# egbariajad/GNN-Accelerated-LAP-Warm-Start-Pipeline

Measured on AMD Instinct MI355X. Metric: LAP instances/sec (whole node), n=2048 warm-start pipeline, higher is better.
Workload: dtype f64

## Files before the change

gnn-accelerated-lap-warm-start-pipeline_amd/csrc/device_utils.hpp:

```cpp
#pragma once

#include <hip/hip_runtime.h>
#include <stdint.h>

namespace lapwarm {

constexpr int kWave = 64;
constexpr int kMaxWaves = 16;
constexpr double kLarge = 1000000.0;

constexpr int kFlagHasViolation = 1;
constexpr int kFlagInfeasible = 2;
constexpr int kFlagProjected = 4;

__device__ __forceinline__ void pin(double &x) { asm volatile("" : "+v"(x)); }

__device__ __forceinline__ int lo32(double x) { return (int)(__double_as_longlong(x) & 0xffffffffLL); }
__device__ __forceinline__ int hi32(double x) { return (int)(__double_as_longlong(x) >> 32); }
__device__ __forceinline__ double mk_f64(int lo, int hi)
{
    return __longlong_as_double(((long long)hi << 32) | (unsigned int)lo);
}

__device__ __forceinline__ int uni(int x) { return __builtin_amdgcn_readfirstlane(x); }
// ... 47 lines not shown
__device__ __forceinline__ double readlane_f64(double x, int l)
{
    const long long b = __double_as_longlong(x);
    const int lo = __builtin_amdgcn_readlane((int)(b & 0xffffffffLL), l);
    const int hi = __builtin_amdgcn_readlane((int)(b >> 32), l);
    return __longlong_as_double(((long long)hi << 32) | (unsigned int)lo);
}
__device__ __forceinline__ double readlane(double x, int l) { return readlane_f64(x, l); }

struct Top2 {
    double a1;
    int i1;
    double a2;
    int i2;
};

__device__ __forceinline__ Top2 top2_empty()
{
    Top2 t;
    t.a1 = pos_inf();
    t.i1 = 0x7fffffff;
    t.a2 = pos_inf();
    t.i2 = 0x7fffffff;
    return t;
}

__device__ __forceinline__ void top2_push(Top2 &t, double a, int i)
{
    const bool first = pair_less(a, i, t.a1, t.i1);
    const bool second = pair_less(a, i, t.a2, t.i2);
    const double n2a = first ? t.a1 : (second ? a : t.a2);
    const int n2i = first ? t.i1 : (second ? i : t.i2);
    t.a1 = first ? a : t.a1;
    t.i1 = first ? i : t.i1;
    t.a2 = n2a;
    t.i2 = n2i;
}

__device__ __forceinline__ Top2 top2_merge(Top2 p, Top2 q)
{
    const bool qf = pair_less(q.a1, q.i1, p.a1, p.i1);
    const double fa = qf ? q.a1 : p.a1;
    const int fi = qf ? q.i1 : p.i1;
    const double la = qf ? p.a1 : q.a1;
    const int li = qf ? p.i1 : q.i1;
    const double sa = qf ? q.a2 : p.a2;
    const int si = qf ? q.i2 : p.i2;
    const bool ls = pair_less(la, li, sa, si);
    Top2 r;
    r.a1 = fa;
    r.i1 = fi;
    r.a2 = ls ? la : sa;
    r.i2 = ls ? li : si;
    return r;
}


template <class Op>
__device__ __forceinline__ typename Op::T wave_reduce(typename Op::T v)
{
    v = Op::combine(dpp_move<kDppRowShr1, 0xf>(Op::identity(), v), v);
    v = Op::combine(dpp_move<kDppRowShr2, 0xf>(Op::identity(), v), v);
    v = Op::combine(dpp_move<kDppRowShr4, 0xf>(Op::identity(), v), v);
    v = Op::combine(dpp_move<kDppRowShr8, 0xf>(Op::identity(), v), v);
    v = Op::combine(dpp_move<kDppRowBcast15, 0xa>(Op::identity(), v), v);
    v = Op::combine(dpp_move<kDppRowBcast31, 0xc>(Op::identity(), v), v);
    return readlane(v, kWave - 1);
}

template <class Op>
__device__ __forceinline__ typename Op::T row_reduce(typename Op::T v)
{
    v = Op::combine(dpp_move<kDppRowShr1, 0xf>(Op::identity(), v), v);
    v = Op::combine(dpp_move<kDppRowShr2, 0xf>(Op::identity(), v), v);
    v = Op::combine(dpp_move<kDppRowShr4, 0xf>(Op::identity(), v), v);
    v = Op::combine(dpp_move<kDppRowShr8, 0xf>(Op::identity(), v), v);
    return readlane(v, 15);
}

struct MinF64 {
    using T = double;
    static __device__ __forceinline__ T identity() { return pos_inf(); }
    static __device__ __forceinline__ T combine(T o, T v) { return dmin(v, o); }
};
struct NanMinF64 : MinF64 {
    static __device__ __forceinline__ T combine(T o, T v) { return nmin(v, o); }
};
struct FminF64 : MinF64 {
    static __device__ __forceinline__ T combine(T o, T v) { return __builtin_fmin(v, o); }
};
struct MaxF64 {
    using T = double;
    static __device__ __forceinline__ T identity() { return -pos_inf(); }
    static __device__ __forceinline__ T combine(T o, T v) { return (o > v) ? o : v; }
};
struct MinI32 {
    using T = int;
    static __device__ __forceinline__ T identity() { return 0x7fffffff; }
    static __device__ __forceinline__ T combine(T o, T v) { return (o < v) ? o : v; }
};
struct SumI32 {
    using T = int;
    static __device__ __forceinline__ T identity() { return 0; }
    static __device__ __forceinline__ T combine(T o, T v) { return v + o; }
};
struct MinU64 {
    using T = unsigned long long;
    static __device__ __forceinline__ T identity() { return ~0ull; }
    static __device__ __forceinline__ T combine(T o, T v) { return (o < v) ? o : v; }
};
__device__ __forceinline__ unsigned f32_key(float x)
{
    if (x != x) return 0xffffffffu;
    unsigned b = __float_as_uint(x);
    if (b == 0x80000000u) b = 0u;
    return (b & 0x80000000u) ? ~b : (b | 0x80000000u);
}

__device__ __forceinline__ double wave_min(double v) { return wave_reduce<MinF64>(v); }
__device__ __forceinline__ double wave_max(double v) { return wave_reduce<MaxF64>(v); }
__device__ __forceinline__ int wave_min_i32(int v) { return wave_reduce<MinI32>(v); }
__device__ __forceinline__ int wave_sum_i32(int v) { return wave_reduce<SumI32>(v); }

template <int CTRL, int ROW_MASK>
__device__ __forceinline__ Top2 top2_step(Top2 t)
{
    Top2 o;
    o.a1 = dpp_move<CTRL, ROW_MASK>(pos_inf(), t.a1);
    o.i1 = dpp_move<CTRL, ROW_MASK>(0x7fffffff, t.i1);
    o.a2 = dpp_move<CTRL, ROW_MASK>(pos_inf(), t.a2);
    o.i2 = dpp_move<CTRL, ROW_MASK>(0x7fffffff, t.i2);
    return top2_merge(t, o);
}
__device__ __forceinline__ Top2 wave_top2(Top2 t)
{
    t = top2_step<kDppRowShr1, 0xf>(t);
    t = top2_step<kDppRowShr2, 0xf>(t);
    t = top2_step<kDppRowShr4, 0xf>(t);
    t = top2_step<kDppRowShr8, 0xf>(t);
    t = top2_step<kDppRowBcast15, 0xa>(t);
    t = top2_step<kDppRowBcast31, 0xc>(t);
    Top2 r;
    r.a1 = readlane_f64(t.a1, kWave - 1);
    r.i1 = __builtin_amdgcn_readlane(t.i1, kWave - 1);
    r.a2 = readlane_f64(t.a2, kWave - 1);
    r.i2 = __builtin_amdgcn_readlane(t.i2, kWave - 1);
    return r;
}

__device__ __forceinline__ double wave_sum_f64(double v)
{
#pragma unroll
    for (int m = 32; m >= 1; m >>= 1) v += __shfl_xor(v, m, kWave);
    return v;
}

template <int CTRL, int ROW_MASK>
__device__ __forceinline__ void scan_step_min_pair(double &v, int &i)
{
    const double ov = dpp_move<CTRL, ROW_MASK>(pos_inf(), v);
    const int oi = dpp_move<CTRL, ROW_MASK>(0x7fffffff, i);
    if (pair_less(ov, oi, v, i)) {
        v = ov;
        i = oi;
    }
}

__device__ __forceinline__ void wave_excl_prefix_min_pair(double &v, int &idx, int lane, double *tv, int *ti)
{
    double iv = v;
    int ii = idx;
    scan_step_min_pair<kDppRowShr1, 0xf>(iv, ii);
    scan_step_min_pair<kDppRowShr2, 0xf>(iv, ii);
    scan_step_min_pair<kDppRowShr4, 0xf>(iv, ii);
    scan_step_min_pair<kDppRowShr8, 0xf>(iv, ii);
    scan_step_min_pair<kDppRowBcast15, 0xa>(iv, ii);
    scan_step_min_pair<kDppRowBcast31, 0xc>(iv, ii);
    {
        const long long b = __double_as_longlong(iv);
        const int lo = __builtin_amdgcn_readlane((int)(b & 0xffffffffLL), kWave - 1);
        const int hi = __builtin_amdgcn_readlane((int)(b >> 32), kWave - 1);
        *tv = __longlong_as_double(((long long)hi << 32) | (unsigned int)lo);
        *ti = __builtin_amdgcn_readlane(ii, kWave - 1);
    }
    const double pv = __shfl_up(iv, 1, kWave);
    const int pi = __shfl_up(ii, 1, kWave);
    v = (lane == 0) ? pos_inf() : pv;
    idx = (lane == 0) ? 0x7fffffff : pi;
}

struct BlockExchange {
    double d[2][kMaxWaves * 4];
    double bcast[2];
    int i[2][kMaxWaves * 4];
};

struct Arr2 {
    double a1, vj1, a2;
    int i1, y1, i2, y2;
};

__device__ __forceinline__ Arr2 arr2_empty()
{
    Arr2 t;
    t.a1 = t.a2 = pos_inf();
    t.vj1 = 0.0;
    t.i1 = t.i2 = 0x7fffffff;
    t.y1 = t.y2 = -1;
    return t;
}

__device__ __forceinline__ void arr2_push(Arr2 &t, double a, int i, double vj, int yj)
{
    const bool first = pair_less(a, i, t.a1, t.i1);
    const bool second = pair_less(a, i, t.a2, t.i2);
    t.a2 = first ? t.a1 : (second ? a : t.a2);
    t.i2 = first ? t.i1 : (second ? i : t.i2);
    t.y2 = first ? t.y1 : (second ? yj : t.y2);
    t.a1 = first ? a : t.a1;
    t.i1 = first ? i : t.i1;
    t.vj1 = first ? vj : t.vj1;
    t.y1 = first ? yj : t.y1;
}

template <int WIDTH>
__device__ __forceinline__ double lanes_min(double v)
{
    static_assert(WIDTH == 64 || WIDTH == 16, "a whole wave or one row");
    if constexpr (WIDTH == 64)
        return wave_reduce<MinF64>(v);
    else
        return row_reduce<MinF64>(v);
}

template <int WIDTH>
__device__ __forceinline__ Arr2 arr2_reduce_lanes(const Arr2 &t)
{
    constexpr int last = WIDTH - 1;
    const unsigned long long lanes = (WIDTH == 64) ? ~0ull : 0xffffull;
    const double m1 = lanes_min<WIDTH>(t.a1);
    const unsigned long long k1 = __ballot(t.a1 == m1) & lanes;
    const int l1 = k1 ? __builtin_ctzll(k1) : 0;
    Arr2 r;
    r.a1 = readlane_f64(t.a1, l1);
    r.vj1 = readlane_f64(t.vj1, l1);
    r.i1 = __builtin_amdgcn_readlane(t.i1, l1);
    r.y1 = __builtin_amdgcn_readlane(t.y1, l1);
    const int lane = threadIdx.x & (kWave - 1);
    const double c2 = ((lane & last) == l1) ? t.a2 : t.a1;
    const int c2i = ((lane & last) == l1) ? t.i2 : t.i1;
    const int c2y = ((lane & last) == l1) ? t.y2 : t.y1;
    const double m2 = lanes_min<WIDTH>(c2);
    const unsigned long long k2 = __ballot(c2 == m2) & lanes;
    const int l2 = k2 ? __builtin_ctzll(k2) : 0;
    r.a2 = readlane_f64(c2, l2);
    r.i2 = __builtin_amdgcn_readlane(c2i, l2);
    r.y2 = __builtin_amdgcn_readlane(c2y, l2);
    return r;
}

struct BlockCtx {
    int tid, lane, wave, nwaves;
    int parity;
    BlockExchange *ex;

    __device__ __forceinline__ void init(BlockExchange *e)
    {
        tid = threadIdx.x;
        lane = tid & (kWave - 1);
        wave = tid >> 6;
        nwaves = (blockDim.x + kWave - 1) >> 6;
        parity = 0;
        ex = e;
    }

    __device__ __forceinline__ double &slot(int p, int w, double) { return ex->d[p][w]; }
    __device__ __forceinline__ int &slot(int p, int w, int) { return ex->i[p][w]; }
    __device__ __forceinline__ unsigned long long &slot(int p, int w, unsigned long long)
    {
        return reinterpret_cast<unsigned long long &>(ex->d[p][w]);
    }

    template <class Op>
    __device__ __forceinline__ typename Op::T reduce(typename Op::T v)
    {
        v = wave_reduce<Op>(v);
        const int p = parity;
        parity ^= 1;
        if (lane == 0) slot(p, wave, v) = v;
        __syncthreads();
        const int w = lane & (kMaxWaves - 1);
        return row_reduce<Op>((w < nwaves) ? slot(p, w, v) : Op::identity());
    }

    template <class Op = MinF64>
    __device__ __forceinline__ double min_f64(double v) { return reduce<Op>(v); }
    __device__ __forceinline__ int min_i32(int v) { return reduce<MinI32>(v); }
    __device__ __forceinline__ int sum_i32(int v) { return reduce<SumI32>(v); }

    __device__ __forceinline__ double max_f64(double v)
    {
        v = wave_max(v);
        const int p = parity;
        parity ^= 1;
        if (lane == 0) ex->d[p][wave] = v;
        __syncthreads();
// ... 136 lines not shown
```

gnn-accelerated-lap-warm-start-pipeline_amd/csrc/jv_solver.hip:

```cpp
#include <string.h>

#include "device_utils.hpp"
#include "jv_solver.hpp"
#include "solve_plan.hpp"

namespace lapwarm {

namespace {

struct EventSlot {
    int j, p, i, a;
};

constexpr int kRecEvents = 4;

struct alignas(16) Ctrl {
    double level;
    int hi;
    int target;
    alignas(16) EventSlot rec[2][kRecEvents];
    alignas(16) int a_pub[2][kRecEvents];
    int tie_find;
    int ev_total[2];
    int first_fire;
    int nfree;
    int err;
    int head_j, head_i;
    int free_pos[2];
};
struct ArrState {
    unsigned arr_current, arr_rr;
    int arr_new_free, arr_fwd, arr_iters, arr_fast, arr_err;
};
static_assert(sizeof(ArrState) <= sizeof(EventSlot) * 2 * kRecEvents, "ArrState is overlaid on Ctrl::rec");

constexpr int kSentinelIdx = 0x7ffffffe;
constexpr int kEmptyIdx = 0x7fffffff;

#ifdef LAPWARM_STAMPS
__device__ __forceinline__ unsigned long long stamp_now()
{
    unsigned long long t;
    asm volatile("s_memtime %0\n\ts_waitcnt lgkmcnt(0)" : "=s"(t)::"memory");
    return t;
}
#ifndef LAPWARM_STAMP_GROUPS
#define LAPWARM_STAMP_GROUPS 7
#endif
#define STAMP_G(g, var) const unsigned long long var = ((LAPWARM_STAMP_GROUPS) & (g)) ? stamp_now() : 0ull
#ifndef LAPWARM_FIND_MASK
#define LAPWARM_FIND_MASK 0x1ff
#endif
#define STAMP_FI(bit, var) const unsigned long long var = (((LAPWARM_STAMP_GROUPS) & 1) && ((LAPWARM_FIND_MASK) >> (bit) & 1)) ? stamp_now() : 0ull
#define STAMP(var) STAMP_G(1, var)
#define STAMPR(var) STAMP_G(2, var)
#define STAMPP(var) STAMP_G(4, var)
#define STAMP_ADD(slot, t1, t0) stamps[slot] += (long long)((t1) - (t0))
#define STAMP_INC(slot) stamps[slot] += 1
#else
#define STAMP(var)
#define STAMPR(var)
#define STAMPP(var)
#define STAMP_FI(bit, var)
#define STAMP_ADD(slot, t1, t0)
#define STAMP_INC(slot)
#endif

template <int CH, int LDSL, int TB, bool RAGGED = false>
struct Solver {
    static constexpr bool LDS_STATE = LDSL > 0 && LDSL != 8;
    static constexpr bool ROWLDS = LDSL == 8;
    static constexpr bool PF = ROWLDS;
    static constexpr int kCacheLimit = (TB <= 256) ? 16 : ((TB <= 512) ? 32 : 4);
    static constexpr int kCacheLimitY = (TB <= 256) ? 16 : 2;
    const double *C;
    int n, W;
    int ldc;
    double *dist, *v;
    int *order, *pred, *y, *x, *fr;
    int *ring;
    int ring_count;
    unsigned char *slots;
    int slot_bytes;
    int nslots;
    uint32_t *evt, *sbits, *used;
    uint32_t *evb;
    int Wpad;
    int *evl;
    int *tmpcol;
    Ctrl *ctrl;
    BlockCtx bc;
    long long scan_elems, init_elems, colred_elems;
    int paths, finds, scan_steps, arr_iters, transfer_rows, arr_fired;
    int step_id;
    int ctrl_seen0, ctrl_seen1, ctrl_find_seq;
    int err;
#ifdef LAPWARM_STAMPS
    long long stamps[kStampSlots];
#endif

    __device__ __forceinline__ int base() const { return bc.tid * CH; }

    __device__ __forceinline__ void ring_push(int row)
    {
        if (ring && (unsigned)row < (unsigned)n) {
            if (bc.tid == 0) {
                const int gen = (ring_count >> 6) + 1;
                __hip_atomic_store(&ring[2 + (ring_count & (kRingSlots - 1))], (gen << 16) | row, __ATOMIC_RELAXED,
                                   __HIP_MEMORY_SCOPE_AGENT);
            }
            ++ring_count;
        }
    }
    __device__ __forceinline__ void ring_push_scan(int lo, int hi)
    {
        if (!ring) return;
        int cnt = hi - lo - 1;
        if (cnt <= 0) return;
        cnt = (cnt < kRingSlots - 2) ? cnt : kRingSlots - 2;
        if (bc.wave == 0 && bc.lane < cnt) {
            const int j = order[lo + 1 + bc.lane];
            const int i = ((unsigned)j < (unsigned)n) ? y[j] : -1;
            const int c = ring_count + bc.lane;
            const int gen = (c >> 6) + 1;
            const int word = (gen << 16) | (((unsigned)i < (unsigned)n) ? i : 0xffff);
            __hip_atomic_store(&ring[2 + (c & (kRingSlots - 1))], word, __ATOMIC_RELAXED, __HIP_MEMORY_SCOPE_AGENT);
        }
        ring_count += cnt;
    }

    __device__ __forceinline__ void fence_if_global()
    {
        if constexpr (!LDS_STATE) __threadfence_block();
    }

    __device__ __forceinline__ void replay_find(int lo)
    {
        const int lane = bc.lane;
        const int wpl = (W + kWave - 1) / kWave;
        int mine = 0;
        for (int q = 0; q < wpl; ++q) {
            const int idx = lane * wpl + q;
            if (idx < W) mine += __popc(evt[idx]);
        }
        int incl = mine;
#pragma unroll
        for (int off = 1; off < kWave; off <<= 1) {
            const int o = __shfl_up(incl, off, kWave);
            if (lane >= off) incl += o;
        }
        const int E = __shfl(incl, kWave - 1, kWave);
        int slot = incl - mine;
        int last_strict_local = -1;
        for (int q = 0; q < wpl; ++q) {
            const int idx = lane * wpl + q;
            if (idx < W) {
                uint32_t ew = evt[idx];
                const uint32_t sw = sbits[idx];
                if (ew) {
                    evt[idx] = 0;
                    sbits[idx] = 0;
                }
                while (ew) {
                    const int bit = __builtin_ctz(ew);
                    ew &= ew - 1;
                    const int st = (sw >> bit) & 1u;
                    if (st) last_strict_local = slot;
                    evl[slot++] = ((idx << 5) + bit) | (st << 31);
                }
            }
        }
        int L = last_strict_local;
#pragma unroll
        for (int m = 32; m >= 1; m >>= 1) {
            const int o = __shfl_xor(L, m, kWave);
            L = (o > L) ? o : L;
        }
        bool early_tie = false;
        for (int i = lane; i < L; i += kWave) early_tie |= (evl[i] >= 0);
        int hi;
        if (__ballot(early_tie) != 0ull || L + 1 > kWave) {
            hi = lo + 1;
            for (int i = 0; i < E; ++i) {
                const int ev = evl[i];
                const int k = ev & 0x7fffffff;
                const int j = order[k];
                if (ev < 0) hi = lo;
                const int a = order[hi];
                if (lane == 0) {
                    order[k] = a;
                    order[hi] = j;
                }
                fence_if_global();
                ++hi;
            }
        } else {
            const int T = E - (L + 1);
            for (int base_i = 0; base_i <= L; base_i += kWave) {
                const int i = base_i + lane;
                int newcol = 0, e = 0;
                if (i <= L) {
                    e = evl[i] & 0x7fffffff;
                    newcol = order[(i == 0) ? lo : (evl[i - 1] & 0x7fffffff)];
                }
                const int lastcol = (L >= 0) ? order[evl[L] & 0x7fffffff] : 0;
                if (i <= L) order[e] = newcol;
                if (base_i == 0 && L >= 0 && lane == 0) order[lo] = lastcol;
            }
            fence_if_global();
            const int tb = L + 1;
            for (int s0 = 1; s0 <= T; s0 += kWave) {
                const int sidx = s0 + lane;
                if (sidx <= T) tmpcol[sidx] = order[evl[tb + sidx - 1] & 0x7fffffff];
            }
            fence_if_global();
            for (int s0 = 1; s0 <= T; s0 += kWave) {
                const int sidx = s0 + lane;
                if (sidx <= T) {
                    const int p0 = lo + sidx;
                    int tpos = evl[tb + sidx - 1] & 0x7fffffff;
                    bool is_tie;
                    {
                        int lo_i = 1, hi_i = sidx;
                        while (lo_i < hi_i) {
                            const int mid = (lo_i + hi_i) >> 1;
                            if ((evl[tb + mid - 1] & 0x7fffffff) < p0)
                                lo_i = mid + 1;
                            else
                                hi_i = mid;
                        }
                        is_tie = ((evl[tb + lo_i - 1] & 0x7fffffff) == p0);
                    }
                    if (!is_tie) {
                        const int col = order[p0];
                        int p = tpos;
                        int guard = 0;
                        while (p <= lo + T && guard++ < n) p = evl[tb + (p - lo) - 1] & 0x7fffffff;
                        order[p] = col;
                    }
                }
            }
            fence_if_global();
            for (int s0 = 1; s0 <= T; s0 += kWave) {
                const int sidx = s0 + lane;
                if (sidx <= T) order[lo + sidx] = tmpcol[sidx];
            }
            fence_if_global();
            hi = lo + 1 + T;
        }
        int best = -1;
        for (int kk = lo + lane; kk < hi; kk += kWave) {
            if (y[order[kk]] < 0) best = kk;
        }
#pragma unroll
        for (int m = 32; m >= 1; m >>= 1) {
            const int o = __shfl_xor(best, m, kWave);
            best = (o > best) ? o : best;
        }
        const int target = (best >= 0) ? order[best] : -1;
        const int head_j = order[lo];
        const double level = dist[head_j];
        const int head_i = y[head_j];
        if (lane == 0) {
            ctrl->hi = hi;
            ctrl->target = target;
            ctrl->level = level;
            ctrl->head_j = head_j;
            ctrl->head_i = head_i;
        }
    }

    __device__ __forceinline__ void replay_scan(int hi, int par)
    {
        const int lane = bc.lane;
        uint32_t *evb = this->evb + (size_t)par * Wpad;
        int target = -1;
        const int fp = uni(ctrl->free_pos[par]);
        if (fp != 0x7fffffff && lane == 0) ctrl->free_pos[par] = 0x7fffffff;
        for (int wbase = 0; wbase < W; wbase += kWave) {
            const int idx = wbase + lane;
            uint32_t ew = 0;
            if (idx < W) {
                ew = evb[idx];
                if (ew) evb[idx] = 0;
            }
            unsigned long long mask = __ballot(ew != 0);
            while (mask && target < 0) {
                const int l = __builtin_ctzll(mask);
                mask &= mask - 1;
                uint32_t e = __shfl(ew, l, kWave);
                while (e && target < 0) {
                    const int bit = __builtin_ctz(e);
                    e &= e - 1;
                    const int k = ((wbase + l) << 5) + bit;
                    const int j = order[k];
                    if (k == fp) {
                        target = j;
                    } else {
                        const int a = order[hi];
                        if (lane == 0) {
                            order[k] = a;
                            order[hi] = j;
                        }
                        fence_if_global();
                        ++hi;
                    }
                }
            }
        }
        if (lane == 0) {
            ctrl->hi = hi;
            ctrl->target = target;
        }
    }

    __device__ __forceinline__ int find_path(int start)
    {
        const int b0 = base();
        const int wordi = b0 >> 5, shift = b0 & 31;
        STAMPP(tpath);
        constexpr bool CACHE_V = CH <= kCacheLimit;
        double dk[CH], vr[CACHE_V ? CH : 1];
        constexpr bool CACHE_Y = CH <= kCacheLimitY;
        int jr[CH], yr[CACHE_Y ? CH : 1];
        {
            const double *row = C + (size_t)start * (RAGGED ? ldc : n);
            double c0[CH];
#pragma unroll
            for (int r = 0; r < CH; ++r) {
                const int k = b0 + r;
                jr[r] = (k < n) ? k : n - 1;
                c0[r] = row[jr[r]];
            }
#pragma unroll
            for (int r = 0; r < CH; ++r) pin(c0[r]);
#pragma unroll
            for (int r = 0; r < CH; ++r) {
                const int k = b0 + r;
                const double vk = v[jr[r]];
                if constexpr (CACHE_V) {
                    vr[r] = vk;
                    if constexpr (CACHE_Y) yr[r] = y[jr[r]];
                }
                const double val = c0[r] - vk;
                dk[r] = (k < n) ? val : pos_inf();
                if (k < n) {
                    order[k] = k;
                    pred[k] = start;
                    dist[k] = val;
                }
            }
        }
        paths++;
        init_elems += n;
        int lo = 0, hi = 0, ready = 0, target = -1;
        int head_j = 0, head_i = 0;
        STAMPP(tp0);
        STAMP_ADD(8, tp0, tpath);
        int seen0 = ctrl_seen0, seen1 = ctrl_seen1;
        int find_seq = ctrl_find_seq;
        int app_pos = -1, app_j = 0, app_i = 0, app_j1 = 0, app_i1 = 0;
        bool app_two = false;
        constexpr bool kFastMulti = CH <= 4;
        bool pf_have = false;
        int pf_slot = 0;
        double level = 0.0;
        int guard = 0;
        while (target < 0) {
            if (lo == hi) {
                STAMP_FI(0, tf0);
                ready = lo;
                ++find_seq;
                double tv = pos_inf();
                int tp = 0x7fffffff;
#pragma unroll
                for (int r = 0; r < CH; ++r) {
                    const int k = b0 + r;
                    if (k >= lo && k < n && (k == lo || dk[r] < tv)) {
                        tv = dk[r];
                        tp = k;
                    }
                }
                double runv = tv, wtv;
                int runp = tp, wtp;
                wave_excl_prefix_min_pair(runv, runp, bc.lane, &wtv, &wtp);
                const int xp = bc.parity;
                bc.parity ^= 1;
                if (bc.lane == 0) {
                    bc.ex->d[xp][bc.wave] = wtv;
                    bc.ex->i[xp][bc.wave] = wtp;
                }
                STAMP_FI(1, tfa);
                STAMP_ADD(9, tfa, tf0);
                __syncthreads();
                STAMP_FI(2, tfb);
                STAMP_ADD(10, tfb, tfa);
                double totv;
                int totp;
                {
                    const int w = bc.lane & (kMaxWaves - 1);
                    double av = (w < bc.nwaves) ? bc.ex->d[xp][w] : pos_inf();
                    int ap = (w < bc.nwaves) ? bc.ex->i[xp][w] : 0x7fffffff;
                    scan_step_min_pair<kDppRowShr1, 0xf>(av, ap);
                    scan_step_min_pair<kDppRowShr2, 0xf>(av, ap);
                    scan_step_min_pair<kDppRowShr4, 0xf>(av, ap);
                    scan_step_min_pair<kDppRowShr8, 0xf>(av, ap);
                    totv = readlane_f64(av, kMaxWaves - 1);
                    totp = __builtin_amdgcn_readlane(ap, kMaxWaves - 1);
                    if (bc.wave > 0) {
                        const int wl = uni(bc.wave) - 1;
                        const double pv = readlane_f64(av, wl);
                        const int pp = __builtin_amdgcn_readlane(ap, wl);
                        if (pair_less(pv, pp, runv, runp)) {
                            runv = pv;
                            runp = pp;
                        }
                    }
                }
                STAMP_FI(3, tfc);
                uint32_t eb = 0, sb = 0;
                bool tie = false;
                int prevpos[CH];
                double prevval[CH];
#pragma unroll
                for (int r = 0; r < CH; ++r) {
                    const int k = b0 + r;
                    prevpos[r] = -1;
                    prevval[r] = 0.0;
                    if (k >= lo && k < n) {
                        if (k > lo && dk[r] <= runv) {
                            eb |= 1u << r;
                            if (dk[r] < runv) {
                                sb |= 1u << r;
                                prevpos[r] = runp;
                                prevval[r] = runv;
                            } else {
                                tie = true;
                            }
                        }
                        if (k == lo || dk[r] < runv) {
                            runv = dk[r];
                            runp = k;
                        }
                    }
                }
                int prevcol[CH];
#pragma unroll
                for (int r = 0; r < CH; ++r) prevcol[r] = (prevpos[r] >= 0) ? order[prevpos[r]] : 0;
                const int min_col = uni(order[totp]);
                if (tie) ctrl->tie_find = find_seq;
                const int min_row_raw = y[min_col];
                ring_push(uni(min_row_raw));
                STAMP_FI(4, tfd);
                STAMP_ADD(11, tfd, tfc);
                __syncthreads();
                STAMP_FI(5, tfe);
                STAMP_ADD(12, tfe, tfd);
                finds++;
                if (uni(ctrl->tie_find) != find_seq) {
                    hi = lo + 1;
                    level = totv;
                    head_j = min_col;
                    head_i = uni(min_row_raw);
                    target = (head_i < 0) ? head_j : -1;
                    if (target >= 0) break;
#pragma unroll
                    for (int r = 0; r < CH; ++r) {
                        if (sb & (1u << r)) {
                            const int k = b0 + r;
                            order[k] = prevcol[r];
                            jr[r] = prevcol[r];
                            dk[r] = prevval[r];
                            if constexpr (CACHE_V) {
                                vr[r] = v[prevcol[r]];
                                if constexpr (CACHE_Y) yr[r] = y[prevcol[r]];
                            }
                        }
                    }
                    if (totp != lo && lo >= b0 && lo < b0 + CH) order[lo] = min_col;
                    STAMP_FI(6, tff);
                    STAMP_ADD(13, tff, tfe);
                } else {
                    if (eb) {
                        atomicOr(&evt[wordi], eb << shift);
                        if (sb) atomicOr(&sbits[wordi], sb << shift);
                    }
                    __syncthreads();
                    if (bc.wave == 0) replay_find(lo);
                    __syncthreads();
                    hi = uni(ctrl->hi);
                    target = uni(ctrl->target);
                    level = uni(ctrl->level);
                    head_j = uni(ctrl->head_j);
                    head_i = uni(ctrl->head_i);
                    STAMP_FI(7, tfg);
                    STAMP_ADD(14, tfg, tfe);
                    STAMP_INC(15);
                    if (target >= 0) break;
                    ring_push_scan(lo, hi);
#pragma unroll
                    for (int r = 0; r < CH; ++r) {
                        const int k = b0 + r;
                        if (k >= hi && k < n) {
                            const int j = order[k];
                            if (j != jr[r]) {
                                jr[r] = j;
                                if constexpr (CACHE_V) {
                                    vr[r] = v[j];
                                    if constexpr (CACHE_Y) yr[r] = y[j];
                                }
                                dk[r] = dist[j];
                            }
                        }
                    }
                }
                STAMP_FI(8, tf1);
                STAMP_ADD(0, tf1, tf0);
            }
            STAMPR(tr0);
            if ((unsigned)head_i >= (unsigned)n || (unsigned)head_j >= (unsigned)n) {
                err = 6;
                break;
            }
            const double *row = C + (size_t)head_i * (RAGGED ? ldc : n);
            double c[CH];
            double c_head;
            bool from_slot = false;
            if constexpr (PF) from_slot = pf_have;
            if constexpr (ROWLDS) {
                if (!from_slot) {
                    pf_slot = 0;
                    const unsigned sbase = lds_address(slots) + (unsigned)bc.wave * 1024u;
                    const int nt = (int)blockDim.x;
#pragma unroll
                    for (int q = 0; q < CH / 2; ++q) {
                        int col = q * 2 * nt + 2 * bc.tid;
                        col = (col < n - 2) ? col : n - 2;
                        dma_request16(row + col, sbase + (unsigned)q * (unsigned)nt * 16u);
                    }
                    drain();
                    __syncthreads();
                    from_slot = true;
                }
            }
            const double *srow = reinterpret_cast<const double *>(slots + (size_t)pf_slot * slot_bytes);
            if constexpr (ROWLDS) {
                c_head = srow[head_j];
            } else if (from_slot) {
#pragma unroll
                for (int r = 0; r < CH; ++r) {
                    const unsigned jc = umin_u32((unsigned)jr[r], (unsigned)(n - 1));
                    c[r] = srow[jc];
                }
                c_head = srow[head_j];
            } else {
#pragma unroll
                for (int r = 0; r < CH; ++r) {
                    const unsigned jc = umin_u32((unsigned)jr[r], (unsigned)(n - 1));
                    c[r] = row[jc];
                }
                c_head = row[head_j];
            }
            const int par = step_id & 1;
            step_id++;
            scan_steps++;
            scan_elems += (long long)(n - hi);
            if (++guard > 2 * n + 4) {
                err = 1;
                break;
            }
            const bool queued = (lo + 1 < hi);
            int nq_j = 0, nq_i = 0;
            const int fwd_pos = app_pos;
            const bool fwd_two = app_two;
            app_pos = -1;
            app_two = false;
            if (queued) {
                if (fwd_two && lo == fwd_pos) {
                    nq_j = app_j1;
                    nq_i = app_i1;
                } else if (lo + 1 == fwd_pos) {
                    nq_j = app_j;
                    nq_i = app_i;
                } else {
                    nq_j = order[lo + 1];
                    nq_i = y[nq_j];
                }
            }

            bool pf_issued = false;
            int pf_next_slot = 0;
            if constexpr (PF) {
                const int ri = uni(nq_i);
                if (queued && (unsigned)ri < (unsigned)n && nslots > 1) {
                    pf_next_slot = from_slot ? (pf_slot ^ 1) : 0;
                    const double *nrow = C + (size_t)ri * (RAGGED ? ldc : n);
                    const unsigned sbase = lds_address(slots) + (unsigned)pf_next_slot * (unsigned)slot_bytes +
                                           (unsigned)bc.wave * 1024u;
                    const int nt = (int)blockDim.x;
#pragma unroll
                    for (int q = 0; q < CH / 2; ++q) {
                        int col = q * 2 * nt + 2 * bc.tid;
                        col = (col < n - 2) ? col : n - 2;
                        dma_request16(nrow + col, sbase + (unsigned)q * (unsigned)nt * 16u);
                    }
                    pf_issued = true;
                }
            }
            if constexpr (kFastMulti) {
                if (b0 <= hi + kRecEvents - 1 && b0 + CH - 1 >= hi) {
#pragma unroll
                    for (int r = 0; r < CH; ++r) {
                        const unsigned w = (unsigned)(b0 + r - hi);
                        if (w < (unsigned)kRecEvents && b0 + r < n) ctrl->a_pub[par][w] = jr[r];
                    }
                }
            } else {
                if (hi >= b0 && hi < b0 + CH && hi < n) {
#pragma unroll
                    for (int r = 0; r < CH; ++r)
                        if (b0 + r == hi) ctrl->a_pub[par][0] = jr[r];
                }
            }
            const double v_head = v[head_j];
            if constexpr (!ROWLDS) {
#pragma unroll
                for (int r = 0; r < CH; ++r) pin(c[r]);
            }
            pin(c_head);
            STAMPR(tr1);
            STAMP_ADD(1, tr1, tr0);
            const double h = (c_head - v_head) - level;
            int my_events = 0, ev_r = -1;
            unsigned imp_bits = 0, ev_mask = 0;
#pragma unroll
            for (int r = 0; r < CH; ++r) {
                const int k = b0 + r;
                const bool act = (k >= hi) & (k < n);
                double vj;
                if constexpr (CACHE_V)
                    vj = vr[r];
                else
                    vj = v[jr[r]];
                double cr;
                if constexpr (ROWLDS)
                    cr = srow[umin_u32((unsigned)jr[r], (unsigned)(n - 1))];
                else
                    cr = c[r];
                const double cand = (cr - vj) - h;
                const bool imp = act & (cand < dk[r]);
                const bool ev = imp & (cand == level);
                dk[r] = imp ? cand : (act ? dk[r] : pos_inf());
                imp_bits |= imp ? (1u << r) : 0u;
                ev_mask |= ev ? (1u << r) : 0u;
            }
            if (imp_bits) {
#pragma unroll
                for (int r = 0; r < CH; ++r) {
                    if ((imp_bits >> r) & 1u) {
                        dist[jr[r]] = dk[r];
                        pred[jr[r]] = head_i;
                    }
                }
                if (ev_mask) {
#pragma unroll
                    for (int r = CH - 1; r >= 0; --r) {
                        if ((ev_mask >> r) & 1u) {
                            ev_r = r;
                            ++my_events;
                            const int k = b0 + r;
                            atomicOr(&evb[par * Wpad + (k >> 5)], 1u << (k & 31));
                            int yj;
                            if constexpr (CACHE_Y)
                                yj = yr[r];
                            else
                                yj = y[jr[r]];
                            if (yj < 0) atomicMin(&ctrl->free_pos[par], k);
                        }
                    }
                }
            }
            const int seen = par ? seen1 : seen0;
            if (my_events && !kFastMulti) {
                atomicAdd(&ctrl->ev_total[par], my_events);
                EventSlot sl;
                sl.j = 0;
                sl.i = 0;
#pragma unroll
                for (int r = 0; r < CH; ++r) {
                    if (r == ev_r) {
                        sl.j = jr[r];
                        if constexpr (CACHE_Y)
                            sl.i = yr[r];
                        else
                            sl.i = y[jr[r]];
                    }
                }
                sl.p = b0 + ev_r;
                sl.a = 0;
                ctrl->rec[par][0] = sl;
            }
            if (my_events && kFastMulti) {
                int slot_idx = atomicAdd(&ctrl->ev_total[par], my_events) - seen;
#pragma unroll
                for (int r = 0; r < CH; ++r) {
                    if ((ev_mask >> r) & 1u) {
                        if (slot_idx < kRecEvents) {
                            EventSlot sl;
                            sl.j = jr[r];
                            if constexpr (CACHE_Y)
                                sl.i = yr[r];
                            else
                                sl.i = y[jr[r]];
                            sl.p = b0 + r;
                            sl.a = 0;
                            ctrl->rec[par][slot_idx] = sl;
                        }
                        ++slot_idx;
                    }
                }
            }
            STAMPR(tr2);
            STAMP_ADD(2, tr2, tr1);
            if constexpr (PF) {
                if (pf_issued) drain();
                pf_have = pf_issued;
                pf_slot = pf_next_slot;
            }
            __syncthreads();
            STAMPR(tr3);
            STAMP_ADD(3, tr3, tr2);
            const int tot_raw = ctrl->ev_total[par];
            EventSlot sl = ctrl->rec[par][0];
            const int a_raw = ctrl->a_pub[par][0];
            const int tot = uni(tot_raw);
            const int cnt = tot - seen;
            if (par)
                seen1 = tot;
            else
                seen0 = tot;
            if (cnt == 0) {
                STAMP_INC(5);
                ++lo;
                if (queued) {
                    head_j = uni(nq_j);
                    head_i = uni(nq_i);
                }
            } else if (cnt == 1) {
                STAMP_INC(6);
                sl.j = uni(sl.j);
                sl.p = uni(sl.p);
                sl.i = uni(sl.i);
                sl.a = uni(a_raw);
                if ((unsigned)sl.j >= (unsigned)n || (unsigned)sl.a >= (unsigned)n || (unsigned)sl.p >= (unsigned)n ||
                    sl.i >= n) {
                    err = 8;
                    break;
                }
                if (sl.p >= b0 && sl.p < b0 + CH) {
                    evb[par * Wpad + (sl.p >> 5)] = 0;
                    if (sl.i >= 0) {
                        const double va = v[sl.a], da = dist[sl.a];
                        const int ya = y[sl.a];
#pragma unroll
                        for (int r = 0; r < CH; ++r) {
                            if (b0 + r == sl.p) {
                                jr[r] = sl.a;
                                if constexpr (CACHE_V) {
                                    vr[r] = va;
                                    if constexpr (CACHE_Y) yr[r] = ya;
                                }
                                dk[r] = da;
                            }
                        }
                        order[sl.p] = sl.a;
                        order[hi] = sl.j;
                    }
                }
                if (sl.i < 0) {
                    if (bc.tid == 0) ctrl->free_pos[par] = 0x7fffffff;
                    target = sl.j;
                    break;
                }
                app_pos = hi;
                app_j = sl.j;
                app_i = sl.i;
                ring_push(sl.i);
                ++hi;
                ++lo;
                if (queued) {
                    head_j = uni(nq_j);
                    head_i = uni(nq_i);
                } else {
                    head_j = sl.j;
                    head_i = sl.i;
                }
            } else {
                STAMP_INC(7);
                bool resolved = false;
                if (kFastMulti && cnt <= kRecEvents) {
                    const EventSlot e1 = ctrl->rec[par][1];
                    const EventSlot e2 = ctrl->rec[par][2];
                    const EventSlot e3 = ctrl->rec[par][3];
                    const int4 aw = *reinterpret_cast<const int4 *>(ctrl->a_pub[par]);
                    const int fp = ctrl->free_pos[par];
                    const int kNone = 0x7fffffff;
                    const int P0 = sl.p, P1 = e1.p, P2 = (cnt > 2) ? e2.p : kNone, P3 = (cnt > 3) ? e3.p : kNone;
                    int pmin = (P0 < P1) ? P0 : P1;
                    pmin = (P2 < pmin) ? P2 : pmin;
                    pmin = (P3 < pmin) ? P3 : pmin;
                    unsigned bad = ((unsigned)P0 >= (unsigned)n) | ((unsigned)sl.j >= (unsigned)n) | (sl.i >= n) |
                                   ((unsigned)P1 >= (unsigned)n) | ((unsigned)e1.j >= (unsigned)n) | (e1.i >= n);
                    if (cnt > 2) bad |= ((unsigned)P2 >= (unsigned)n) | ((unsigned)e2.j >= (unsigned)n) | (e2.i >= n);
                    if (cnt > 3) bad |= ((unsigned)P3 >= (unsigned)n) | ((unsigned)e3.j >= (unsigned)n) | (e3.i >= n);
                    bad |= (hi + cnt > n);
                    if (uni((int)bad)) {
                        err = 8;
                        break;
                    }
                    if (uni(fp) != kNone) {
                        int tj = -1;
                        tj = (P0 == fp) ? sl.j : tj;
                        tj = (P1 == fp) ? e1.j : tj;
                        tj = (P2 == fp) ? e2.j : tj;
                        tj = (P3 == fp) ? e3.j : tj;
                        tj = uni(tj);
                        if (tj >= 0) {
#pragma unroll
                            for (int r = 0; r < CH; ++r)
                                if ((ev_mask >> r) & 1u) atomicAnd(&evb[par * Wpad + ((b0 + r) >> 5)], ~(1u << ((b0 + r) & 31)));
                            target = tj;
                            break;
                        }
                    } else if (uni(pmin) >= hi + cnt) {
                        const int r0 = (P1 < P0) + (P2 < P0) + (P3 < P0);
                        const int r1 = (P0 < P1) + (P2 < P1) + (P3 < P1);
                        const int r2 = (P0 < P2) + (P1 < P2) + (P3 < P2);
                        const int r3 = (P0 < P3) + (P1 < P3) + (P2 < P3);
                        int first_j = sl.j, first_i = sl.i, second_j = sl.j, second_i = sl.i;
                        first_j = (r1 == 0) ? e1.j : first_j, first_i = (r1 == 0) ? e1.i : first_i;
                        first_j = (r2 == 0) ? e2.j : first_j, first_i = (r2 == 0) ? e2.i : first_i;
                        first_j = (r3 == 0) ? e3.j : first_j, first_i = (r3 == 0) ? e3.i : first_i;
                        second_j = (r1 == 1) ? e1.j : second_j, second_i = (r1 == 1) ? e1.i : second_i;
                        second_j = (r2 == 1) ? e2.j : second_j, second_i = (r2 == 1) ? e2.i : second_i;
                        second_j = (r3 == 1) ? e3.j : second_j, second_i = (r3 == 1) ? e3.i : second_i;
                        if (ev_mask) {
#pragma unroll
                            for (int r = 0; r < CH; ++r) {
                                if ((ev_mask >> r) & 1u) {
                                    const int pk = b0 + r;
                                    int rank = r0, jq = sl.j;
                                    rank = (pk == P1) ? r1 : rank, jq = (pk == P1) ? e1.j : jq;
                                    rank = (pk == P2) ? r2 : rank, jq = (pk == P2) ? e2.j : jq;
                                    rank = (pk == P3) ? r3 : rank, jq = (pk == P3) ? e3.j : jq;
                                    int a = aw.x;
                                    a = (rank == 1) ? aw.y : a;
                                    a = (rank == 2) ? aw.z : a;
                                    a = (rank == 3) ? aw.w : a;
                                    if ((unsigned)a >= (unsigned)n || (pk != P0 && pk != P1 && pk != P2 && pk != P3)) {
                                        ctrl->err = 8;
                                    } else {
                                        jr[r] = a;
                                        if constexpr (CACHE_V) {
                                            vr[r] = v[a];
                                            if constexpr (CACHE_Y) yr[r] = y[a];
                                        }
                                        dk[r] = dist[a];
                                        order[pk] = a;
                                        order[hi + rank] = jq;
                                    }
                                    atomicAnd(&evb[par * Wpad + (pk >> 5)], ~(1u << (pk & 31)));
                                }
                            }
                        }
                        app_pos = hi;
                        app_j = uni(first_j);
                        app_i = uni(first_i);
                        app_j1 = uni(second_j);
                        app_i1 = uni(second_i);
                        app_two = true;
                        ring_push(app_i);
                        ring_push(app_i1);
                        if (cnt > 2) {
                            int third_i = sl.i, fourth_i = sl.i;
                            third_i = (r1 == 2) ? e1.i : third_i, third_i = (r2 == 2) ? e2.i : third_i;
                            third_i = (r3 == 2) ? e3.i : third_i;
                            fourth_i = (r1 == 3) ? e1.i : fourth_i, fourth_i = (r2 == 3) ? e2.i : fourth_i;
                            fourth_i = (r3 == 3) ? e3.i : fourth_i;
                            ring_push(uni(third_i));
                            if (cnt > 3) ring_push(uni(fourth_i));
                        }
                        hi += cnt;
                        ++lo;
                        if (queued) {
                            head_j = uni(nq_j);
                            head_i = uni(nq_i);
                        } else {
                            head_j = app_j;
                            head_i = app_i;
                        }
                        resolved = true;
                    }
                }
                if (resolved) {
                    STAMPR(tr4m);
                    STAMP_ADD(4, tr4m, tr3);
                    continue;
                }
                const int hi_before = hi;
                if (bc.wave == 0) replay_scan(hi, par);
                __syncthreads();
                hi = uni(ctrl->hi);
                target = uni(ctrl->target);
                if (target >= 0) break;
                ring_push_scan(hi_before - 1, hi);
                ++lo;
                if (queued) {
                    head_j = uni(nq_j);
                    head_i = uni(nq_i);
                } else {
                    head_j = uni(order[lo]);
                    head_i = uni(y[head_j]);
                }
                if (ev_mask) {
#pragma unroll
                    for (int r = 0; r < CH; ++r) {
                        const int k = b0 + r;
                        if (((ev_mask >> r) & 1u) && k >= hi && k < n) {
                            const int j = order[k];
                            jr[r] = j;
                            if constexpr (CACHE_V) {
                                vr[r] = v[j];
                                if constexpr (CACHE_Y) yr[r] = y[j];
                            }
                            dk[r] = dist[j];
                        }
                    }
                }
            }
            STAMPR(tr4);
            STAMP_ADD(4, tr4, tr3);
        }
        ctrl_seen0 = seen0;
        ctrl_seen1 = seen1;
        ctrl_find_seq = find_seq;
        __syncthreads();
        if (bc.tid == 0) {
            ctrl->free_pos[0] = 0x7fffffff;
            ctrl->free_pos[1] = 0x7fffffff;
        }
#pragma unroll
        for (int r = 0; r < CH; ++r) {
            const int k = b0 + r;
            if (k < ready) {
                const int j = order[k];
                v[j] += dist[j] - level;
            }
        }
        return target;
    }

    __device__ __forceinline__ void augment_all(int f_first, int n_free)
    {
        for (int f = f_first; f < n_free && !err; ++f) {
            const int start = uni(fr[f]);
            if ((unsigned)start >= (unsigned)n) {
                err = 2;
                break;
            }
            if (f + 1 < n_free) ring_push(uni(fr[f + 1]));
            const int target = find_path(start);
            if (err) break;
            if (bc.tid == 0) {
                int j = target, i = -1, hops = 0;
                bool ok = true;
                while (i != start && hops <= n) {
                    if ((unsigned)j >= (unsigned)n) {
                        ok = false;
                        break;
                    }
                    i = pred[j];
                    if ((unsigned)i >= (unsigned)n) {
                        ok = false;
                        break;
                    }
                    y[j] = i;
                    const int prev = x[i];
                    x[i] = j;
                    j = prev;
                    ++hops;
                }
                if (!ok || i != start) ctrl->err = 3;
            }
            __syncthreads();
            if (uni(ctrl->err)) {
                err = 3;
                break;
            }
        }
    }

    __device__ __forceinline__ int cold_column_reduction()
    {
        const int b0 = base();
        double vm[CH];
        int ya[CH];
#pragma unroll
        for (int r = 0; r < CH; ++r) {
            vm[r] = kLarge;
            ya[r] = 0;
        }
        int jc[CH];
#pragma unroll
        for (int r = 0; r < CH; ++r) jc[r] = (b0 + r < n) ? b0 + r : n - 1;
        constexpr int RU = (CH <= 2) ? 8 : ((CH <= 4) ? 4 : 2);
        int i = 0;
        for (; i + RU <= n; i += RU) {
            double c[RU][CH];
#pragma unroll
            for (int q = 0; q < RU; ++q) {
                const double *row = C + (size_t)(i + q) * (RAGGED ? ldc : n);
#pragma unroll
                for (int r = 0; r < CH; ++r) c[q][r] = row[jc[r]];
            }
#pragma unroll
            for (int q = 0; q < RU; ++q) {
#pragma unroll
                for (int r = 0; r < CH; ++r) pin(c[q][r]);
            }
#pragma unroll
            for (int q = 0; q < RU; ++q) {
#pragma unroll
                for (int r = 0; r < CH; ++r) {
                    if (c[q][r] < vm[r]) {
                        vm[r] = c[q][r];
                        ya[r] = i + q;
                    }
                }
            }
        }
        for (; i < n; ++i) {
            const double *row = C + (size_t)i * (RAGGED ? ldc : n);
#pragma unroll
            for (int r = 0; r < CH; ++r) {
                const double c = row[jc[r]];
                if (c < vm[r]) {
                    vm[r] = c;
                    ya[r] = i;
                }
            }
        }
        colred_elems += (long long)n * n;
#pragma unroll
        for (int r = 0; r < CH; ++r) {
            const int j = b0 + r;
            if (j < n) {
                v[j] = vm[r];
                y[j] = ya[r];
                x[j] = -1;
                pred[j] = 0;
            }
        }
        __syncthreads();
#pragma unroll
        for (int r = 0; r < CH; ++r) {
            const int j = b0 + r;
            if (j < n) {
                atomicMax(&x[ya[r]], j);
                atomicAdd(&pred[ya[r]], 1);
            }
        }
        __syncthreads();
#pragma unroll
        for (int r = 0; r < CH; ++r) {
            const int j = b0 + r;
            if (j < n && x[ya[r]] != j) y[j] = -1;
        }
        __syncthreads();
        int nf = 0;
        for (int i = 0; i < n; ++i) {
            const int xi = x[i];
            if (xi < 0) {
                if (bc.tid == 0) fr[nf] = i;
                ++nf;
            } else if (pred[i] == 1) {
                const double *row = C + (size_t)i * (RAGGED ? ldc : n);
                double m = kLarge;
                double ct[CH];
#pragma unroll
                for (int r = 0; r < CH; ++r) ct[r] = row[jc[r]];
// ... 1113 lines not shown
```

Measured before the change: 423.1.

## Resolve multi-event steps from event bitmap with wave prefix-sum ranking

Replaces the fast multi-event path, which was limited to four recorded events and needed per-event slot publishing, with a bitmap-based approach. Each owning thread ranks its event positions via a wave-wide inclusive prefix sum of popcounts and swaps with order[hi+rank] in parallel when all events lie beyond hi+cnt. Otherwise it falls back to a single-wave replay scan that keeps the bits, followed by a barrier. This removes the rec/a_pub publishing work and handles any event count without a serial replay. The cost is an extra barrier on every multi-event step and more global reads of the bitmap. The forwarded second-head bookkeeping is also dropped, and some timing-stamp macros are added.

```diff
diff --git a/gnn-accelerated-lap-warm-start-pipeline_amd/csrc/device_utils.hpp b/gnn-accelerated-lap-warm-start-pipeline_amd/csrc/device_utils.hpp
--- a/gnn-accelerated-lap-warm-start-pipeline_amd/csrc/device_utils.hpp
+++ b/gnn-accelerated-lap-warm-start-pipeline_amd/csrc/device_utils.hpp
@@ -223,6 +223,17 @@
 {
 #pragma unroll
     for (int m = 32; m >= 1; m >>= 1) v += __shfl_xor(v, m, kWave);
+    return v;
+}
+
+__device__ __forceinline__ int wave_incl_prefix_sum_i32(int v)
+{
+    v += dpp_move<kDppRowShr1, 0xf>(0, v);
+    v += dpp_move<kDppRowShr2, 0xf>(0, v);
+    v += dpp_move<kDppRowShr4, 0xf>(0, v);
+    v += dpp_move<kDppRowShr8, 0xf>(0, v);
+    v += dpp_move<kDppRowBcast15, 0xa>(0, v);
+    v += dpp_move<kDppRowBcast31, 0xc>(0, v);
     return v;
 }
 
diff --git a/gnn-accelerated-lap-warm-start-pipeline_amd/csrc/jv_solver.hip b/gnn-accelerated-lap-warm-start-pipeline_amd/csrc/jv_solver.hip
--- a/gnn-accelerated-lap-warm-start-pipeline_amd/csrc/jv_solver.hip
+++ b/gnn-accelerated-lap-warm-start-pipeline_amd/csrc/jv_solver.hip
@@ -12,14 +12,14 @@
     int j, p, i, a;
 };
 
-constexpr int kRecEvents = 4;
+constexpr int kRecStride = 4;
 
 struct alignas(16) Ctrl {
     double level;
     int hi;
     int target;
-    alignas(16) EventSlot rec[2][kRecEvents];
-    alignas(16) int a_pub[2][kRecEvents];
+    alignas(16) EventSlot rec[2][kRecStride];
+    alignas(16) int a_pub[2][kRecStride];
     int tie_find;
     int ev_total[2];
     int first_fire;
@@ -32,7 +32,7 @@
     unsigned arr_current, arr_rr;
     int arr_new_free, arr_fwd, arr_iters, arr_fast, arr_err;
 };
-static_assert(sizeof(ArrState) <= sizeof(EventSlot) * 2 * kRecEvents, "ArrState is overlaid on Ctrl::rec");
+static_assert(sizeof(ArrState) <= sizeof(EventSlot) * 2 * kRecStride, "ArrState is overlaid on Ctrl::rec");
 
 constexpr int kSentinelIdx = 0x7ffffffe;
 constexpr int kEmptyIdx = 0x7fffffff;
@@ -57,6 +57,38 @@
 #define STAMPP(var) STAMP_G(4, var)
 #define STAMP_ADD(slot, t1, t0) stamps[slot] += (long long)((t1) - (t0))
 #define STAMP_INC(slot) stamps[slot] += 1
+#ifdef LAPWARM_STAMP_MULTI
+static_assert((LAPWARM_STAMP_GROUPS) == 2, "the multi-event anatomy reuses the slots of stamp groups 1 and 4");
+#define STAMP_CLASS(cls)                                                           \
+    do {                                                                           \
+        const unsigned long long stamp_class_end = stamp_now();                    \
+        stamps[8 + 2 * (cls)] += (long long)(stamp_class_end - tr3) + (1ll << 40); \
+        stamps[9 + 2 * (cls)] += (long long)(tr3 - tr2);                           \
+    } while (0)
+#define STAMP_CLASS_SWAPPED() STAMP_CLASS(0)
+#define STAMP_CLASS_FREE() STAMP_CLASS(1)
+#define STAMP_CLASS_REPLAYED(cnt) \
+    do {                          \
+        if ((cnt) > 4)            \
+            STAMP_CLASS(2);       \
+        else                      \
+            STAMP_CLASS(3);       \
+    } while (0)
+#define STAMP_EVENTS(cnt)                                                                             \
+    do {                                                                                              \
+        if ((cnt) <= 4)                                                                               \
+            stamps[0] += 1ll << (21 * ((cnt) - 2));                                                   \
+        else                                                                                          \
+            stamps[7] += ((cnt) <= 8) ? 1ll : (1ll << 32);                                            \
+    } while (0)
+#define STAMP_INC_UNLESS_MULTI(slot)
+#else
+#define STAMP_CLASS_SWAPPED()
+#define STAMP_CLASS_FREE()
+#define STAMP_CLASS_REPLAYED(cnt)
+#define STAMP_EVENTS(cnt)
+#define STAMP_INC_UNLESS_MULTI(slot) STAMP_INC(slot)
+#endif
 #else
 #define STAMP(var)
 #define STAMPR(var)
@@ -64,6 +96,11 @@
 #define STAMP_FI(bit, var)
 #define STAMP_ADD(slot, t1, t0)
 #define STAMP_INC(slot)
+#define STAMP_INC_UNLESS_MULTI(slot)
+#define STAMP_CLASS_SWAPPED()
+#define STAMP_CLASS_FREE()
+#define STAMP_CLASS_REPLAYED(cnt)
+#define STAMP_EVENTS(cnt)
 #endif
 
 template <int CH, int LDSL, int TB, bool RAGGED = false>
@@ -270,6 +307,7 @@
         }
     }
 
+    template <bool KEEP_BITS = false>
     __device__ __forceinline__ void replay_scan(int hi, int par)
     {
         const int lane = bc.lane;
@@ -282,7 +320,9 @@
             uint32_t ew = 0;
             if (idx < W) {
                 ew = evb[idx];
-                if (ew) evb[idx] = 0;
+                if constexpr (!KEEP_BITS) {
+                    if (ew) evb[idx] = 0;
+                }
             }
             unsigned long long mask = __ballot(ew != 0);
             while (mask && target < 0) {
@@ -359,8 +399,7 @@
         STAMP_ADD(8, tp0, tpath);
         int seen0 = ctrl_seen0, seen1 = ctrl_seen1;
         int find_seq = ctrl_find_seq;
-        int app_pos = -1, app_j = 0, app_i = 0, app_j1 = 0, app_i1 = 0;
-        bool app_two = false;
+        int app_pos = -1, app_j = 0, app_i = 0;
         constexpr bool kFastMulti = CH <= 4;
         bool pf_have = false;
         int pf_slot = 0;
@@ -495,7 +534,7 @@
                     head_i = uni(ctrl->head_i);
                     STAMP_FI(7, tfg);
                     STAMP_ADD(14, tfg, tfe);
-                    STAMP_INC(15);
+                    STAMP_INC_UNLESS_MULTI(15);
                     if (target >= 0) break;
                     ring_push_scan(lo, hi);
 #pragma unroll
@@ -572,14 +611,9 @@
             const bool queued = (lo + 1 < hi);
             int nq_j = 0, nq_i = 0;
             const int fwd_pos = app_pos;
-            const bool fwd_two = app_two;
             app_pos = -1;
-            app_two = false;
             if (queued) {
-                if (fwd_two && lo == fwd_pos) {
-                    nq_j = app_j1;
-                    nq_i = app_i1;
-                } else if (lo + 1 == fwd_pos) {
+                if (lo + 1 == fwd_pos) {
                     nq_j = app_j;
                     nq_i = app_i;
                 } else {
@@ -607,20 +641,10 @@
                     pf_issued = true;
                 }
             }
-            if constexpr (kFastMulti) {
-                if (b0 <= hi + kRecEvents - 1 && b0 + CH - 1 >= hi) {
-#pragma unroll
-                    for (int r = 0; r < CH; ++r) {
-                        const unsigned w = (unsigned)(b0 + r - hi);
-                        if (w < (unsigned)kRecEvents && b0 + r < n) ctrl->a_pub[par][w] = jr[r];
-                    }
-                }
-            } else {
-                if (hi >= b0 && hi < b0 + CH && hi < n) {
-#pragma unroll
-                    for (int r = 0; r < CH; ++r)
-                        if (b0 + r == hi) ctrl->a_pub[par][0] = jr[r];
-                }
+            if (hi >= b0 && hi < b0 + CH && hi < n) {
+#pragma unroll
+                for (int r = 0; r < CH; ++r)
+                    if (b0 + r == hi) ctrl->a_pub[par][0] = jr[r];
             }
             const double v_head = v[head_j];
             if constexpr (!ROWLDS) {
@@ -681,7 +705,7 @@
                 }
             }
             const int seen = par ? seen1 : seen0;
-            if (my_events && !kFastMulti) {
+            if (my_events) {
                 atomicAdd(&ctrl->ev_total[par], my_events);
                 EventSlot sl;
                 sl.j = 0;
@@ -699,26 +723,6 @@
                 sl.p = b0 + ev_r;
                 sl.a = 0;
                 ctrl->rec[par][0] = sl;
-            }
-            if (my_events && kFastMulti) {
-                int slot_idx = atomicAdd(&ctrl->ev_total[par], my_events) - seen;
-#pragma unroll
-                for (int r = 0; r < CH; ++r) {
-                    if ((ev_mask >> r) & 1u) {
-                        if (slot_idx < kRecEvents) {
-                            EventSlot sl;
-                            sl.j = jr[r];
-                            if constexpr (CACHE_Y)
-                                sl.i = yr[r];
-                            else
-                                sl.i = y[jr[r]];
-                            sl.p = b0 + r;
-                            sl.a = 0;
-                            ctrl->rec[par][slot_idx] = sl;
-                        }
-                        ++slot_idx;
-                    }
-                }
             }
             STAMPR(tr2);
             STAMP_ADD(2, tr2, tr1);
@@ -796,123 +800,109 @@
                     head_i = sl.i;
                 }
             } else {
-                STAMP_INC(7);
-                bool resolved = false;
-                if (kFastMulti && cnt <= kRecEvents) {
-                    const EventSlot e1 = ctrl->rec[par][1];
-                    const EventSlot e2 = ctrl->rec[par][2];
-                    const EventSlot e3 = ctrl->rec[par][3];
-                    const int4 aw = *reinterpret_cast<const int4 *>(ctrl->a_pub[par]);
-                    const int fp = ctrl->free_pos[par];
-                    const int kNone = 0x7fffffff;
-                    const int P0 = sl.p, P1 = e1.p, P2 = (cnt > 2) ? e2.p : kNone, P3 = (cnt > 3) ? e3.p : kNone;
-                    int pmin = (P0 < P1) ? P0 : P1;
-                    pmin = (P2 < pmin) ? P2 : pmin;
-                    pmin = (P3 < pmin) ? P3 : pmin;
-                    unsigned bad = ((unsigned)P0 >= (unsigned)n) | ((unsigned)sl.j >= (unsigned)n) | (sl.i >= n) |
-                                   ((unsigned)P1 >= (unsigned)n) | ((unsigned)e1.j >= (unsigned)n) | (e1.i >= n);
-                    if (cnt > 2) bad |= ((unsigned)P2 >= (unsigned)n) | ((unsigned)e2.j >= (unsigned)n) | (e2.i >= n);
-                    if (cnt > 3) bad |= ((unsigned)P3 >= (unsigned)n) | ((unsigned)e3.j >= (unsigned)n) | (e3.i >= n);
-                    bad |= (hi + cnt > n);
-                    if (uni((int)bad)) {
+                STAMP_INC_UNLESS_MULTI(7);
+                STAMP_EVENTS(cnt);
+                bool parallel = false;
+                if constexpr (kFastMulti) {
+                    const int fp = uni(ctrl->free_pos[par]);
+                    if (fp != 0x7fffffff) {
+                        if ((unsigned)fp >= (unsigned)n) {
+                            err = 8;
+                            break;
+                        }
+                        const int tj = uni(order[fp]);
+                        if (ev_mask) atomicAnd(&evb[par * Wpad + wordi], ~(ev_mask << shift));
+                        if ((unsigned)tj >= (unsigned)n) {
+                            err = 8;
+                            break;
+                        }
+                        target = tj;
+                        STAMP_CLASS_FREE();
+                        break;
+                    }
+                    constexpr int kWordsPerLane = (CH * TB > 32 * kWave) ? 2 : 1;
+                    static_assert(CH * TB <= 32 * kWave * kWordsPerLane, "one wave holds the whole event bitmap");
+                    uint32_t wv[kWordsPerLane];
+                    int nbits = 0;
+#pragma unroll
+                    for (int q = 0; q < kWordsPerLane; ++q) {
+                        const int idx = bc.lane * kWordsPerLane + q;
+                        wv[q] = (idx < W) ? evb[par * Wpad + idx] : 0u;
+                        nbits += __popc(wv[q]);
+                    }
+                    const unsigned long long holders = __ballot(nbits != 0);
+                    if (holders == 0ull || hi + cnt > n) {
                         err = 8;
                         break;
                     }
-                    if (uni(fp) != kNone) {
-                        int tj = -1;
-                        tj = (P0 == fp) ? sl.j : tj;
-                        tj = (P1 == fp) ? e1.j : tj;
-                        tj = (P2 == fp) ? e2.j : tj;
-                        tj = (P3 == fp) ? e3.j : tj;
-                        tj = uni(tj);
-                        if (tj >= 0) {
-#pragma unroll
-                            for (int r = 0; r < CH; ++r)
-                                if ((ev_mask >> r) & 1u) atomicAnd(&evb[par * Wpad + ((b0 + r) >> 5)], ~(1u << ((b0 + r) & 31)));
-                            target = tj;
-                            break;
-                        }
-                    } else if (uni(pmin) >= hi + cnt) {
-                        const int r0 = (P1 < P0) + (P2 < P0) + (P3 < P0);
-                        const int r1 = (P0 < P1) + (P2 < P1) + (P3 < P1);
-                        const int r2 = (P0 < P2) + (P1 < P2) + (P3 < P2);
-                        const int r3 = (P0 < P3) + (P1 < P3) + (P2 < P3);
-                        int first_j = sl.j, first_i = sl.i, second_j = sl.j, second_i = sl.i;
-                        first_j = (r1 == 0) ? e1.j : first_j, first_i = (r1 == 0) ? e1.i : first_i;
-                        first_j = (r2 == 0) ? e2.j : first_j, first_i = (r2 == 0) ? e2.i : first_i;
-                        first_j = (r3 == 0) ? e3.j : first_j, first_i = (r3 == 0) ? e3.i : first_i;
-                        second_j = (r1 == 1) ? e1.j : second_j, second_i = (r1 == 1) ? e1.i : second_i;
-                        second_j = (r2 == 1) ? e2.j : second_j, second_i = (r2 == 1) ? e2.i : second_i;
-                        second_j = (r3 == 1) ? e3.j : second_j, second_i = (r3 == 1) ? e3.i : second_i;
+                    const int first_lane = uni(__builtin_ctzll(holders));
+                    int first_pos;
+                    {
+                        const uint32_t f0 = (uint32_t)readlane((int)wv[0], first_lane);
+                        first_pos = first_lane * kWordsPerLane * 32 + __builtin_ctz(f0 | 0x80000000u);
+                        if constexpr (kWordsPerLane == 2) {
+                            const uint32_t f1 = (uint32_t)readlane((int)wv[1], first_lane);
+                            if (f0 == 0u) first_pos = (first_lane * 2 + 1) * 32 + __builtin_ctz(f1 | 0x80000000u);
+                        }
+                    }
+                    parallel = first_pos >= hi + cnt;
+                    if (parallel && __ballot(ev_mask != 0) != 0ull) {
+                        const int below_lane = wave_incl_prefix_sum_i32(nbits) - nbits;
+                        const int src = wordi / kWordsPerLane;
+                        int below = __shfl(below_lane, src, kWave);
+                        uint32_t myw = (uint32_t)__shfl((int)wv[0], src, kWave);
+                        if constexpr (kWordsPerLane == 2) {
+                            const uint32_t w1 = (uint32_t)__shfl((int)wv[1], src, kWave);
+                            if (wordi & 1) {
+                                below += __popc(myw);
+                                myw = w1;
+                            }
+                        }
                         if (ev_mask) {
 #pragma unroll
                             for (int r = 0; r < CH; ++r) {
                                 if ((ev_mask >> r) & 1u) {
                                     const int pk = b0 + r;
-                                    int rank = r0, jq = sl.j;
-                                    rank = (pk == P1) ? r1 : rank, jq = (pk == P1) ? e1.j : jq;
-                                    rank = (pk == P2) ? r2 : rank, jq = (pk == P2) ? e2.j : jq;
-                                    rank = (pk == P3) ? r3 : rank, jq = (pk == P3) ? e3.j : jq;
-                                    int a = aw.x;
-                                    a = (rank == 1) ? aw.y : a;
-                                    a = (rank == 2) ? aw.z : a;
-                                    a = (rank == 3) ? aw.w : a;
-                                    if ((unsigned)a >= (unsigned)n || (pk != P0 && pk != P1 && pk != P2 && pk != P3)) {
+                                    const int rank = below + __popc(myw & ((1u << (pk & 31)) - 1u));
+                                    if ((unsigned)rank >= (unsigned)cnt) {
                                         ctrl->err = 8;
                                     } else {
-                                        jr[r] = a;
-                                        if constexpr (CACHE_V) {
-                                            vr[r] = v[a];
-                                            if constexpr (CACHE_Y) yr[r] = y[a];
+                                        const int a = order[hi + rank];
+                                        if ((unsigned)a >= (unsigned)n) {
+                                            ctrl->err = 8;
+                                        } else {
+                                            const int jq = jr[r];
+                                            jr[r] = a;
+                                            if constexpr (CACHE_V) {
+                                                vr[r] = v[a];
+                                                if constexpr (CACHE_Y) yr[r] = y[a];
+                                            }
+                                            dk[r] = dist[a];
+                                            order[pk] = a;
+                                            order[hi + rank] = jq;
                                         }
-                                        dk[r] = dist[a];
-                                        order[pk] = a;
-                                        order[hi + rank] = jq;
                                     }
-                                    atomicAnd(&evb[par * Wpad + (pk >> 5)], ~(1u << (pk & 31)));
                                 }
                             }
                         }
-                        app_pos = hi;
-                        app_j = uni(first_j);
-                        app_i = uni(first_i);
-                        app_j1 = uni(second_j);
-                        app_i1 = uni(second_i);
-                        app_two = true;
-                        ring_push(app_i);
-                        ring_push(app_i1);
-                        if (cnt > 2) {
-                            int third_i = sl.i, fourth_i = sl.i;
-                            third_i = (r1 == 2) ? e1.i : third_i, third_i = (r2 == 2) ? e2.i : third_i;
-                            third_i = (r3 == 2) ? e3.i : third_i;
-                            fourth_i = (r1 == 3) ? e1.i : fourth_i, fourth_i = (r2 == 3) ? e2.i : fourth_i;
-                            fourth_i = (r3 == 3) ? e3.i : fourth_i;
-                            ring_push(uni(third_i));
-                            if (cnt > 3) ring_push(uni(fourth_i));
-                        }
-                        hi += cnt;
-                        ++lo;
-                        if (queued) {
-                            head_j = uni(nq_j);
-                            head_i = uni(nq_i);
-                        } else {
-                            head_j = app_j;
-                            head_i = app_i;
-                        }
-                        resolved = true;
-                    }
-                }
-                if (resolved) {
-                    STAMPR(tr4m);
-                    STAMP_ADD(4, tr4m, tr3);
-                    continue;
+                    }
                 }
                 const int hi_before = hi;
-                if (bc.wave == 0) replay_scan(hi, par);
-                __syncthreads();
-                hi = uni(ctrl->hi);
-                target = uni(ctrl->target);
-                if (target >= 0) break;
+                if constexpr (kFastMulti) {
+                    if (!parallel && bc.wave == 0) replay_scan<true>(hi, par);
+                    __syncthreads();
+                    if (ev_mask) atomicAnd(&evb[par * Wpad + wordi], ~(ev_mask << shift));
+                    hi = parallel ? hi + cnt : uni(ctrl->hi);
+                } else {
+                    if (bc.wave == 0) replay_scan(hi, par);
+                    __syncthreads();
+                    hi = uni(ctrl->hi);
+                    target = uni(ctrl->target);
+                    if (target >= 0) {
+                        STAMP_CLASS_FREE();
+                        break;
+                    }
+                }
                 ring_push_scan(hi_before - 1, hi);
                 ++lo;
                 if (queued) {
@@ -922,7 +912,7 @@
                     head_j = uni(order[lo]);
                     head_i = uni(y[head_j]);
                 }
-                if (ev_mask) {
+                if (!parallel && ev_mask) {
 #pragma unroll
                     for (int r = 0; r < CH; ++r) {
                         const int k = b0 + r;
@@ -936,6 +926,11 @@
                             dk[r] = dist[j];
                         }
                     }
+                }
+                if (parallel) {
+                    STAMP_CLASS_SWAPPED();
+                } else {
+                    STAMP_CLASS_REPLAYED(cnt);
                 }
             }
             STAMPR(tr4);
```

Result: faster. 441.0 (median of 6 runs) (+4.2%).
